# cheneeheng/2s-AGCN

Measured on AMD Instinct MI355X. Metric: skeleton-clips/sec fwd+bwd, NTU (N,3,300,25,2), higher is better.
Workload: dtype f32; 1 GPU; AGCN joint-stream NTU-xview shape, full training step (fwd, CE, bwd, grad all-reduce, clip 1.0, SGD nesterov); per_gpu_batch=64, global_batch=64, input=(N,3,300,25,2), parallelism=dp1, bn=per-replica

## Files before the change

2s-agcn_amd/csrc/adj_fused.hip:

```cpp
#include "agcn_common.h"
#include "split_f16.h"
#include "split_bf16.h"

namespace {

constexpr int CK = 16, NW = 8, NT = 512, WLR = 264, TP = 257;
constexpr int B_BYTES = 3 * 2 * WLR * 16;

struct AfArgs {
  const float* x;
  const unsigned short* wp;
  const float* bias;
  float* spart;
  float* tp_out;
  const float* dS;
  float* dtp;
  float* dbpart;
  int N, C, Ci, T, V, tt, ntiles, nchunks, nsb;
  int npl;
  int dbg;
  unsigned* x_absmax;
};

struct AfPackArgs {
  const float* w;
  unsigned short* wp;
  int M, K, nchunks;
};

template <int BM>
__global__ void __launch_bounds__(256) af_pack_kernel(const AfPackArgs p) {
  constexpr int PER_PLANE = 2 * BM * 8;
  const int ch = blockIdx.x % p.nchunks, sb = blockIdx.x / p.nchunks;
  unsigned short* dst = p.wp + (long)blockIdx.x * 3 * PER_PLANE;
  for (int e = threadIdx.x; e < PER_PLANE / 2; e += 256) {
    const int j = (e & 3) * 2;
    const int ml = (e >> 2) % BM;
    const int h = (e >> 2) / BM;
    const int m = sb * BM + ml;
    float v[2];
#pragma unroll
    for (int q = 0; q < 2; ++q) {
      const int kc = ch * CK + h * 8 + j + q;
      v[q] = (m < p.M && kc < p.K) ? p.w[(long)m * p.K + kc] : 0.f;
    }
    unsigned ph, pm, pl;
    sb_split_pair(v[0], v[1], ph, pm, pl);
    const int o = (h * BM + ml) * 8 + j;
    *reinterpret_cast<unsigned*>(dst + 0 * PER_PLANE + o) = ph;
    *reinterpret_cast<unsigned*>(dst + 1 * PER_PLANE + o) = pm;
    *reinterpret_cast<unsigned*>(dst + 2 * PER_PLANE + o) = pl;
  }
}

template <int TM, int NSUB, int MODE, int PD>
// ... 284 lines not shown
  const size_t stage = 2 * (a_bytes + B_BYTES);
  const int VP = 2 * ((V + 1) / 2);
  const size_t aux_f = (size_t)NW * V * V, aux_b = (size_t)2 * VP * 32 + 32;
  const size_t ph2 = ((size_t)32 * TP + (aux_f > aux_b ? aux_f : aux_b)) * 4;
  g.smem_bytes = ((stage > ph2 ? stage : ph2) + 15) & ~(size_t)15;
  g.pack_bytes = (size_t)g.nsb * g.nchunks * a_bytes;
  return g;
}

inline bool af_shape(int Ci, int& tm, int& nsub) {
  if (Ci == 16) { tm = 3; nsub = 3; return true; }
  if (Ci == 32) { tm = 2; nsub = 1; return true; }
  if (Ci == 64) { tm = 4; nsub = 1; return true; }
  return false;
}

template <int TM, int NSUB, int MODE, int PD>
int af_launch(AfArgs a, const AfGeom& g, hipStream_t s) {
  return agcn_launch_big<adj_fused_kernel<TM, NSUB, MODE, PD>>(dim3((unsigned)(a.N * g.ntiles * g.nsb)), dim3(NT),
                                                               g.smem_bytes, s, a);
}

template <int TM, int NSUB>
int af_pack(const float* wab, void* ws, int M, int K, const AfGeom& g, hipStream_t s) {
  AfPackArgs pk;
  pk.w = wab; pk.wp = (unsigned short*)ws; pk.M = M; pk.K = K; pk.nchunks = g.nchunks;
  hipLaunchKernelGGL((af_pack_kernel<TM * 32>), dim3(g.nsb * g.nchunks), dim3(256), 0, s, pk);
  return agcn_check_launch();
}

template <int TM, int NSUB>
int af_go(int mode, const AfArgs& a, const float* wab, void* ws, const AfGeom& g, hipStream_t s) {
  int rc = af_pack<TM, NSUB>(wab, ws, 6 * a.Ci, a.C, g, s);
  if (rc) return rc;
  const int pd = (g.nchunks % 4 == 0 && (TM <= 2 || g.nchunks >= 8)) ? 4 : (g.nchunks % 2 == 0 ? 2 : 1);
  if (pd == 4) return mode == 0 ? af_launch<TM, NSUB, 0, 4>(a, g, s) : af_launch<TM, NSUB, 1, 4>(a, g, s);
  if (pd == 2) return mode == 0 ? af_launch<TM, NSUB, 0, 2>(a, g, s) : af_launch<TM, NSUB, 1, 2>(a, g, s);
  return mode == 0 ? af_launch<TM, NSUB, 0, 1>(a, g, s) : af_launch<TM, NSUB, 1, 1>(a, g, s);
}

int af_run(int mode, AfArgs a, const float* wab, void* ws, size_t ws_bytes, hipStream_t s) {
  int tm, nsub;
  if (!af_shape(a.Ci, tm, nsub)) return AGCN_ERR_UNSUPPORTED;
  const AfGeom g = af_geometry(a.C, a.T, a.V, tm * 32, nsub);
  if (g.smem_bytes > 160 * 1024) return AGCN_ERR_UNSUPPORTED;
  if (g.pack_bytes > ws_bytes) return AGCN_ERR_WORKSPACE;
  a.tt = g.tt; a.ntiles = g.ntiles; a.nchunks = g.nchunks; a.nsb = g.nsb;
  a.wp = (const unsigned short*)ws;
  a.dbg = agcn_probe(AGCN_AF_DBG, nullptr);
  a.npl = agcn_npl();
  if (tm == 3) return af_go<3, 3>(mode, a, wab, ws, g, s);
  if (tm == 2) return af_go<2, 1>(mode, a, wab, ws, g, s);
  return af_go<4, 1>(mode, a, wab, ws, g, s);
}

bool af_supported(int C, int Ci, int T, int V) {
// ... 17 lines not shown
}

int agcn_adjacency_fused_fwd(const float* x, const float* wab, const float* bab, const float* A, const float* PA,
                             const float* alpha, float* tp_out, float* spart, float* P, float* adj, void* workspace,
                             size_t workspace_bytes, int N, int C, int Ci, int T, int V, void* stream) {
  return agcn_adjacency_fused_fwd_ex(x, wab, bab, A, PA, alpha, tp_out, spart, P, adj, nullptr, nullptr, workspace,
                                     workspace_bytes, N, C, Ci, T, V, stream);
}
int agcn_adjacency_fused_fwd_ex(const float* x, const float* wab, const float* bab, const float* A, const float* PA,
                                const float* alpha, float* tp_out, float* spart, float* P, float* adj, float* x_absmax_out,
                                const float* x_absmax_in, void* workspace, size_t workspace_bytes, int N, int C, int Ci, int T,
                                int V, void* stream) {
  if (!x || !wab || !PA || !spart || !P || !adj || !workspace || N <= 0 || C <= 0 || Ci <= 0 || T <= 0 || V <= 0 ||
      V > 32)
    return AGCN_ERR_ARG;
  if (!af_supported(C, Ci, T, V)) return AGCN_ERR_UNSUPPORTED;
  if (agcn_adj_ws_supported(N, C, Ci, T, V)) {
    const size_t img = agcn_adj_ws_workspace(C, Ci);
    if (workspace_bytes < img + 16) return AGCN_ERR_WORKSPACE;
    hipStream_t s = (hipStream_t)stream;
    const float* amax;
    void* slot = x_absmax_out ? (void*)x_absmax_out : static_cast<char*>(workspace) + img;
    if (int rc = agcn_operand_max(x_absmax_in, x, (long)N * C * T * V, slot, s, &amax)) return rc;
    if (x_absmax_in && x_absmax_out && x_absmax_out != x_absmax_in)
      if (hipMemcpyAsync(x_absmax_out, x_absmax_in, 4, hipMemcpyDeviceToDevice, s) != hipSuccess) return AGCN_ERR_ARG;
    const int tt = 256 / V > T ? T : 256 / V, slots = (T + tt - 1) / tt;
    int nused = 0;
    if (int rc = agcn_adj_ws_scores(x, wab, bab, tp_out, spart, slots, &nused, amax, workspace, img, N, C, Ci, T, V, s))
      return rc;
    return agcn_adj_finalize(spart, A, PA, alpha, P, adj, N, Ci, T, V, s, nused);
  }
  if (x_absmax_out && hipMemsetAsync(x_absmax_out, 0, 4, (hipStream_t)stream) != hipSuccess) return AGCN_ERR_ARG;
  AfArgs a = {};
  a.x_absmax = reinterpret_cast<unsigned*>(x_absmax_out);
  a.x = x; a.bias = bab; a.spart = spart; a.tp_out = tp_out;
  a.N = N; a.C = C; a.Ci = Ci; a.T = T; a.V = V;
  int rc = af_run(0, a, wab, workspace, workspace_bytes, (hipStream_t)stream);
  if (rc) return rc;
  return agcn_adj_finalize(spart, A, PA, alpha, P, adj, N, Ci, T, V, (hipStream_t)stream);
}

int agcn_adjacency_fused_bwd_scores(const float* x, const float* wab, const float* bab, const float* dS, float* dtp,
                                    float* dbpart, void* scratch, float* db, void* workspace, size_t workspace_bytes,
                                    int N, int C, int Ci, int T, int V, void* stream) {
  if (!x || !wab || !dS || !dtp || !dbpart || !scratch || !db || !workspace || N <= 0 || C <= 0 || Ci <= 0 ||
      T <= 0 || V <= 0 || V > 32)
    return AGCN_ERR_ARG;
  if (!af_supported(C, Ci, T, V)) return AGCN_ERR_UNSUPPORTED;
  AfArgs a = {};
  a.x = x; a.bias = bab; a.dS = dS; a.dtp = dtp; a.dbpart = dbpart;
  a.N = N; a.C = C; a.Ci = Ci; a.T = T; a.V = V;
  int rc = af_run(1, a, wab, workspace, workspace_bytes, (hipStream_t)stream);
  if (rc) return rc;
  const int tt = 256 / V > T ? T : 256 / V;
  return agcn_colsum(dbpart, N * ((T + tt - 1) / tt), 6 * Ci, scratch, db, stream);
// ... 4 lines not shown
```

2s-agcn_amd/csrc/adj_ws.hip:

```cpp
#include "agcn_common.h"
#include "split_f16.h"

namespace {

typedef __bf16 bf16x8 __attribute__((ext_vector_type(8)));
typedef unsigned u32x4 __attribute__((ext_vector_type(4)));

constexpr int AW_NW = 8, AW_NT = AW_NW * 64;

struct AwArgs {
  const float* x;
  const unsigned short* wp;
  const float* bias;
  float* spart;
  float* tp_out;
  const float* x_absmax;
  int N, C, Ci, T, V;
  int FT, nsplit, fper, slots;
};

struct AwPackArgs {
  const float* w;
  unsigned short* wp;
  int M, K, nks;
};

__global__ void __launch_bounds__(256) aw_pack_kernel(const AwPackArgs p) {
  const int e = blockIdx.x * 256 + threadIdx.x;
  if (e >= p.nks * 2 * p.M) return;
  const int m = e % p.M, h = (e / p.M) & 1, ks = e / (2 * p.M);
  u32x4 ph, pl;
#pragma unroll
  for (int e2 = 0; e2 < 4; ++e2) {
    float v[2];
#pragma unroll
    for (int q = 0; q < 2; ++q) {
      const int k = 16 * ks + 8 * h + 2 * e2 + q;
      v[q] = k < p.K ? p.w[(long)m * p.K + k] : 0.f;
    }
    unsigned a, b;
    split_pair_f16(v[0] * F16_W_SCALE, v[1] * F16_W_SCALE, a, b);
    ph[e2] = a; pl[e2] = b;
  }
  u32x4* dst = reinterpret_cast<u32x4*>(p.wp);
  dst[((long)(ks * 2 + 0) * 2 + h) * p.M + m] = ph;
  dst[((long)(ks * 2 + 1) * 2 + h) * p.M + m] = pl;
}

template <int TMS, int KS, int NSR, int TP>
__global__ void __launch_bounds__(AW_NT, 2) adj_ws_kernel(const AwArgs a) {
  constexpr int TM = 3 * TMS;
// ... 208 lines not shown
  AGCN_NOTE_KERNEL("adj_ws_kernel<%d, %d, %d, %d>", TMS, KS, NSR, TP);
  return rc;
}
template <int TMS, int KS, int NSR>
int aw_launch(const AwArgs& a, const AwGeom& g, hipStream_t s) {
  return g.TP == 252 ? aw_launch_tp<TMS, KS, NSR, 252>(a, g, s) : aw_launch_tp<TMS, KS, NSR, 256>(a, g, s);
}

}

static inline bool aw_enabled() {
  return agcn_knob(AGCN_ADJ_WS) != 0 && agcn_chain_f16x3();
}

bool agcn_adj_ws_supported(int N, int C, int Ci, int T, int V) {
  AwGeom g;
  return aw_enabled() && aw_geometry(N, C, Ci, T, V, g);
}

size_t agcn_adj_ws_workspace(int C, int Ci) { return (size_t)((C + 15) / 16) * 2 * 2 * (6 * Ci) * 16; }

int agcn_adj_ws_scores(const float* x, const float* wab, const float* bab, float* tp_out, float* spart, int slots,
                       int* nslots_used, const float* x_absmax, void* ws, size_t ws_bytes, int N, int C, int Ci, int T, int V,
                       hipStream_t s) {
  AwGeom g;
  if (!aw_geometry(N, C, Ci, T, V, g)) return AGCN_ERR_UNSUPPORTED;
  if (g.nsplit > slots) return AGCN_ERR_UNSUPPORTED;
  if (g.pack_bytes > ws_bytes) return AGCN_ERR_WORKSPACE;
  AwPackArgs pk;
  pk.w = wab; pk.wp = (unsigned short*)ws; pk.M = 6 * Ci; pk.K = C; pk.nks = g.ks;
  const int items = g.ks * 2 * 6 * Ci;
  hipLaunchKernelGGL(aw_pack_kernel, dim3((items + 255) / 256), dim3(256), 0, s, pk);
  int rc = agcn_check_launch();
  if (rc) return rc;
  AwArgs a = {};
  a.x = x; a.wp = (const unsigned short*)ws; a.bias = bab; a.spart = spart; a.tp_out = tp_out; a.x_absmax = x_absmax;
  a.N = N; a.C = C; a.Ci = Ci; a.T = T; a.V = V;
  a.FT = g.FT; a.nsplit = g.nsplit; a.fper = g.fper; a.slots = slots;
  *nslots_used = g.nsplit;
  if (g.tms == 1 && g.ks == 4) return g.nsr == 3 ? aw_launch<1, 4, 3>(a, g, s) : aw_launch<1, 4, 1>(a, g, s);
  if (g.tms == 2 && g.ks == 4) return aw_launch<2, 4, 1>(a, g, s);
  if (g.tms == 2 && g.ks == 8) return aw_launch<2, 8, 1>(a, g, s);
  return AGCN_ERR_UNSUPPORTED;
}
```

2s-agcn_amd/csrc/agcn_common.h:

```cpp
#pragma once
#include <hip/hip_runtime.h>
#include <stdint.h>
#include <stdlib.h>
#include <string.h>
#include "knobs.h"
#include "../../include/agcn_hip.h"

typedef float f32x16 __attribute__((ext_vector_type(16)));
typedef float f32x4 __attribute__((ext_vector_type(4)));

__device__ __forceinline__ f32x16 mfma32(float a, float b, f32x16 c) {
  return __builtin_amdgcn_mfma_f32_32x32x2f32(a, b, c, 0, 0, 0);
}
__device__ __forceinline__ int mfma_row(int j, int h) { return (j & 3) + 8 * (j >> 2) + 4 * h; }

__device__ __forceinline__ float mask_load(const float* m, long idx, int bits) {
  return bits ? m[idx >> 5] : m[idx];
}
__device__ __forceinline__ bool mask_pass(float raw, long idx, int bits) {
  return bits ? ((__builtin_bit_cast(unsigned, raw) >> (idx & 31)) & 1u) != 0u : raw > 0.f;
}

__device__ __forceinline__ float half_sum(float v) {
  v += __shfl_xor(v, 16);
  v += __shfl_xor(v, 8);
  v += __shfl_xor(v, 4);
  v += __shfl_xor(v, 2);
  v += __shfl_xor(v, 1);
  return v;
}

__device__ __forceinline__ int xcd_remap(int bid, int nwg) {
  const int q = nwg >> 3, r = nwg & 7, x = bid & 7, k = bid >> 3;
  const int base = (x < r) ? x * (q + 1) : r * (q + 1) + (x - r) * q;
  return base + k;
}

int agcn_adj_finalize(const float* spart, const float* A, const float* PA, const float* alpha, float* P, float* adj,
                      int N, int Ci, int T, int V, hipStream_t s, int nused = -1);

bool agcn_adj_ws_supported(int N, int C, int Ci, int T, int V);
size_t agcn_adj_ws_workspace(int C, int Ci);
int agcn_adj_ws_scores(const float* x, const float* wab, const float* bab, float* tp_out, float* spart, int slots,
                       int* nslots_used, const float* x_absmax, void* ws, size_t ws_bytes, int N, int C, int Ci, int T, int V,
                       hipStream_t s);

struct AgcnDryRun {
  long slab_slots;
  size_t ws_bytes;
};
static inline int agcn_dry_note(AgcnDryRun* d, long slab_slots, size_t ws_bytes) {
  if (slab_slots > d->slab_slots) d->slab_slots = slab_slots;
  if (ws_bytes > d->ws_bytes) d->ws_bytes = ws_bytes;
  return AGCN_OK;
}

static inline float* agcn_dry_present() { static float placeholder; return &placeholder; }

static inline bool agcn_sizes_ok(int N, int a, int b, int T, int V) {
  return N > 0 && a > 0 && b > 0 && T > 0 && V > 0 && V <= 32;
}

#include "tconv_plan.h"

bool agcn_bf16_conv_wide(int taps, int M);
enum AgcnTconvOp { AGCN_TCONV_FWD, AGCN_TCONV_BWD_DATA };
bool agcn_bf16_tconv_supported(AgcnTconvOp op, int taps, int stride, int pad);
struct GateArgs;
// ... 77 lines not shown
```

2s-agcn_amd/csrc/bn.hip:

```cpp
#include "agcn_common.h"

namespace {

constexpr int RG = 64;

__global__ void __launch_bounds__(256)
colsum_stage1_kernel(const float* __restrict__ X, int nslots, int W, int per_group, double* __restrict__ partial) {
  __shared__ double red[4][64];
  const int col = blockIdx.x * 64 + (threadIdx.x & 63), sub = threadIdx.x >> 6;
  const int g = blockIdx.y;
  const int s_end = min(nslots, (g + 1) * per_group);
  double acc = 0.0;
  if (col < W)
    for (int s = g * per_group + sub; s < s_end; s += 4) acc += (double)X[(long)s * W + col];
  red[sub][threadIdx.x & 63] = acc;
  __syncthreads();
  if (sub == 0 && col < W)
    partial[(long)g * W + col] = red[0][threadIdx.x] + red[1][threadIdx.x] + red[2][threadIdx.x] + red[3][threadIdx.x];
}

__global__ void colsum_stage2_kernel(const double* __restrict__ partial, int W, float* __restrict__ out) {
  const int col = blockIdx.x * blockDim.x + threadIdx.x;
  if (col >= W) return;
  double s = 0.0;
// ... 150 lines not shown
      dz = ((mb[e >> 5] >> (e & 31)) & 1u) ? dz : 0.f;
    }
    s0 += dz;
    s1 += dz * a[q];
    if (HAS2) s2 += dz * b[q];
  }
  s0 = half_sum(s0); s1 = half_sum(s1); s2 = half_sum(s2);
  s0 += __shfl_xor(s0, 32); s1 += __shfl_xor(s1, 32); s2 += __shfl_xor(s2, 32);
  const int wave = threadIdx.x >> 6;
  if ((threadIdx.x & 63) == 0) { red[0][wave] = s0; red[1][wave] = s1; red[2][wave] = s2; }
  __syncthreads();
  if (threadIdx.x < 3) {
    const int k = threadIdx.x;
    part[row * 3 + k] = red[k][0] + red[k][1] + red[k][2] + red[k][3];
  }
}

__global__ void bn_bwd_finalize_kernel(const float* __restrict__ part, int N, int C, double count, float pscale,
                                       const float* __restrict__ gamma1, const float* __restrict__ mean1,
                                       const float* __restrict__ invstd1, const float* __restrict__ gamma2,
                                       const float* __restrict__ mean2, const float* __restrict__ invstd2,
                                       float* __restrict__ coef, float* __restrict__ dgamma1,
                                       float* __restrict__ dbeta1, float* __restrict__ dgamma2,
                                       float* __restrict__ dbeta2) {
  const int c = blockIdx.x * blockDim.x + threadIdx.x;
  if (c >= C) return;
  double s0 = 0.0, s1 = 0.0, s2 = 0.0;
#pragma unroll 8
  for (int n = 0; n < N; ++n) {
    const float* p = part + ((long)n * C + c) * 3;
    s0 += (double)p[0]; s1 += (double)p[1]; s2 += (double)p[2];
  }
  {
    const double is = invstd1[c], mu = mean1[c], g = gamma1[c];
    const double sxh = is * (s1 - mu * s0);
    const double k = g * is;
    coef[0 * C + c] = (float)k;
    coef[1 * C + c] = (float)(-k * is * sxh / count);
    coef[2 * C + c] = (float)(-k * s0 / count + k * is * mu * sxh / count);
    dgamma1[c] = (float)sxh * pscale;
    dbeta1[c] = (float)s0 * pscale;
  }
  if (gamma2) {
    const double is = invstd2[c], mu = mean2[c], g = gamma2[c];
    const double sxh = is * (s2 - mu * s0);
    const double k = g * is;
    coef[3 * C + c] = (float)k;
    coef[4 * C + c] = (float)(-k * is * sxh / count);
// ... 146 lines not shown
  hipStream_t s = (hipStream_t)stream;
  if (y2) hipLaunchKernelGGL(bn_bwd_reduce_kernel<true>, dim3(N * C), dim3(256), 0, s, dout, (const float*)mask,
                             mask_bits, y1, y2, part, P);
  else hipLaunchKernelGGL(bn_bwd_reduce_kernel<false>, dim3(N * C), dim3(256), 0, s, dout, (const float*)mask,
                          mask_bits, y1, y2, part, P);
  return agcn_check_launch();
}

int agcn_bn_bwd_apply(const float* part, int nrows, double count, float param_grad_scale, const float* dout,
                      const void* mask, int mask_bits, const float* y1, const float* gamma1, const float* mean1, const float* invstd1,
                      const float* y2, const float* gamma2, const float* mean2, const float* invstd2, float* coef,
                      float* dy1, float* dgamma1, float* dbeta1, float* dy2, float* dgamma2, float* dbeta2, int N, int C,
                      int P, void* stream) {
  return agcn_bn_bwd_apply_ex(part, nrows, count, param_grad_scale, dout, mask, mask_bits, y1, gamma1, mean1, invstd1, y2,
                              gamma2, mean2, invstd2, coef, dy1, dgamma1, dbeta1, dy2, dgamma2, dbeta2, nullptr, N, C, P,
                              stream);
}

int agcn_bn_bwd_apply_ex(const float* part, int nrows, double count, float param_grad_scale, const float* dout,
                         const void* mask, int mask_bits, const float* y1, const float* gamma1, const float* mean1,
                         const float* invstd1, const float* y2, const float* gamma2, const float* mean2,
                         const float* invstd2, float* coef, float* dy1, float* dgamma1, float* dbeta1, float* dy2,
                         float* dgamma2, float* dbeta2, float* absmax1_out, int N, int C, int P, void* stream) {
  if (absmax1_out && hipMemsetAsync(absmax1_out, 0, 4, (hipStream_t)stream) != hipSuccess) return AGCN_ERR_ARG;
  if (!part || !dout || !y1 || !gamma1 || !mean1 || !invstd1 || !coef || !dy1 || !dgamma1 || !dbeta1 || nrows <= 0)
    return AGCN_ERR_ARG;
  if (y2 && (!gamma2 || !mean2 || !invstd2 || !dy2 || !dgamma2 || !dbeta2)) return AGCN_ERR_ARG;
  const long total = (long)N * C * P;
  if (total % 4 != 0 || total > 0xffffffffL) return AGCN_ERR_UNSUPPORTED;
  hipStream_t s = (hipStream_t)stream;
  hipLaunchKernelGGL(bn_bwd_finalize_kernel, dim3((C + 63) / 64), dim3(64), 0, s, part, nrows, C, count,
                     param_grad_scale, gamma1, mean1, invstd1, y2 ? gamma2 : nullptr, mean2, invstd2, coef, dgamma1,
                     dbeta1, dgamma2, dbeta2);
  int rc = agcn_check_launch();
  if (rc) return rc;
  const unsigned t4 = (unsigned)(total / 4);
  const dim3 g(ew_grid(t4)), b(256);
  if (y2)
    hipLaunchKernelGGL(bn_bwd_apply_kernel<true>, g, b, 0, s, (const float4*)dout, (const float4*)mask, mask_bits,
                       (const float4*)y1, (const float4*)y2, (const float*)coef, (float4*)dy1, (float4*)dy2, t4,
                       (unsigned)P, (unsigned)C, (unsigned*)absmax1_out);
  else
    hipLaunchKernelGGL(bn_bwd_apply_kernel<false>, g, b, 0, s, (const float4*)dout, (const float4*)mask, mask_bits,
                       (const float4*)y1, (const float4*)y2, (const float*)coef, (float4*)dy1, (float4*)dy2, t4,
                       (unsigned)P, (unsigned)C, (unsigned*)absmax1_out);
  return agcn_check_launch();
}

int agcn_bn_bwd(const float* dout, const void* mask, int mask_bits, const float* y1, const float* gamma1,
                const float* mean1, const float* invstd1, const float* y2, const float* gamma2, const float* mean2,
                const float* invstd2, float* part, float* coef, float* dy1, float* dgamma1, float* dbeta1, float* dy2,
                float* dgamma2, float* dbeta2, int N, int C, int P, void* stream) {
  int rc = agcn_bn_bwd_reduce(dout, mask, mask_bits, y1, y2, part, N, C, P, stream);
  if (rc) return rc;
  return agcn_bn_bwd_apply(part, N, (double)N * (double)P, 1.0f, dout, mask, mask_bits, y1, gamma1, mean1, invstd1, y2, gamma2,
                           mean2, invstd2, coef, dy1, dgamma1, dbeta1, dy2, dgamma2, dbeta2, N, C, P, stream);
// ... 7 lines not shown
```

2s-agcn_amd/csrc/wgrad9_bf16.hip:

```cpp
#include "agcn_common.h"
#include "split_bf16.h"
#include "split_f16.h"

namespace {

constexpr int TC = 80;
constexpr int DP = 84;
constexpr int XW = TC + 8;
constexpr int XPB = 88;

struct TrArgs {
  const float* in;
  float* out;
  int N, R, T, V, Tp, S;
  const float* absmax;
  long plane;
};

template <bool F16, int RB, int TT, int FPL>
__global__ void __launch_bounds__(256) tv_transpose_kernel(const TrArgs a) {
  extern __shared__ __attribute__((aligned(16))) float tile[];
  static_assert(FPL == 4 || (F16 && FPL == 8), "a lane writes one 16-byte store per plane");
  constexpr int QL = TT / FPL, NSUB = 64 / QL;
  const int S = a.S;
  const int ntt = (a.Tp * S + TT - 1) / TT, nrb = (a.R + RB - 1) / RB;
// ... 49 lines not shown
        const int f = (FPL * q + j) * S + par;
        val[j] = (f < tl) ? tile[r * pitch + f * a.V + v] : 0.f;
      }
      const long o = ((((long)n * a.V + v) * a.R + r0 + r) * S + par) * a.Tp + t0 / S + FPL * q;
      if constexpr (F16) {
        unsigned hh[FPL / 2], ll[FPL / 2];
#pragma unroll
        for (int j = 0; j < FPL / 2; ++j) split_pair_f16_mix(val[2 * j] * rs_s, val[2 * j + 1] * rs_s, hh[j], ll[j]);
        unsigned short* oh = reinterpret_cast<unsigned short*>(a.out);
        if constexpr (FPL == 8) {
          *reinterpret_cast<u32x4*>(oh + o) = u32x4{hh[0], hh[1], hh[2], hh[3]};
          *reinterpret_cast<u32x4*>(oh + a.plane + o) = u32x4{ll[0], ll[1], ll[2], ll[3]};
        } else {
          *reinterpret_cast<uint2*>(oh + o) = make_uint2(hh[0], hh[1]);
          *reinterpret_cast<uint2*>(oh + a.plane + o) = make_uint2(ll[0], ll[1]);
        }
      } else {
        *reinterpret_cast<f32x4*>(a.out + o) = f32x4{val[0], val[1], val[2], val[3]};
      }
    }
  }
}

struct W9Args {
  const float* dyT;
  const float* xT;
  float* part;
  int N, M, C, V, T, Tp;
  int nchunk, units, units_per_split, ncb;
  int npl;
  const unsigned short* dyH;
  const unsigned short* xH;
  long dy_plane, x_plane;
  const float* dy_absmax;
  const float* x_absmax;
};

template <int S>
__device__ __forceinline__ bf16x8 window_frag(const unsigned (&p)[8]) {
  u32x4 r;
  if (S % 2 == 0) {
#pragma unroll
    for (int i = 0; i < 4; ++i) r[i] = p[S / 2 + i];
  } else {
#pragma unroll
    for (int i = 0; i < 4; ++i) r[i] = __builtin_amdgcn_alignbit(p[(S + 1) / 2 + i], p[(S - 1) / 2 + i], 16);
// ... 329 lines not shown
inline W9Geom w9_geometry(int N, int M, int C, int V, int T, int stride, int taps = 9, int Tx = 0) {
  W9Geom g;
  g.rt = (M % 128 == 0) ? 4 : 2;
  const int BM = g.rt * 32, CBW = (4 / g.rt) * 32;
  g.Tp = ((Tx > T ? Tx : T) + 7) & ~7;
  g.nchunk = (T + TC - 1) / TC;
  g.units = N * V * g.nchunk;
  g.nmb = (M + BM - 1) / BM;
  g.ncb = (C + CBW - 1) / CBW;
  const int tiles = g.nmb * g.ncb;
  int want = 512 / tiles;
  if (want < 1) want = 1;
  if (want > g.units) want = g.units;
  g.units_per_split = (g.units + want - 1) / want;
  g.nsplit = (g.units + g.units_per_split - 1) / g.units_per_split;
  g.slab_bytes = (size_t)g.nsplit * taps * M * C * 4;
  g.dyT_bytes = (size_t)N * V * M * g.Tp * 4;
  g.xT_bytes = (size_t)N * V * C * stride * g.Tp * 4;
  g.smem_bytes = (size_t)BM * DP * 4 + (size_t)3 * stride * CBW * XPB * 2;
  g.smem_f16 = (size_t)2 * BM * DPH * 2 + (size_t)2 * stride * CBW * XPB * 2;
  return g;
}

int w9_transpose(const float* in, float* out, int N, int R, int T, int V, int Tp, int S, hipStream_t s,
                 const float* absmax = nullptr) {
  TrArgs t;
  t.in = in; t.out = out; t.N = N; t.R = R; t.T = T; t.V = V; t.Tp = Tp; t.S = S;
  t.absmax = absmax; t.plane = (long)N * V * R * S * Tp;
  if (absmax) {
    const int rem = T % 128;
    if (T <= 128 || rem == 0 || rem > 64) {
      constexpr int RB = 4, TT = 128;
      const int ntt = (Tp * S + TT - 1) / TT, nrb = (R + RB - 1) / RB;
      const size_t smem = (size_t)RB * (TT * V + 4) * 4;
      hipLaunchKernelGGL((tv_transpose_kernel<true, RB, TT, 8>), dim3((unsigned)(N * nrb * ntt)), dim3(256), smem, s, t);
    } else {
      constexpr int RB = 8, TT = 64;
      const int ntt = (Tp * S + TT - 1) / TT, nrb = (R + RB - 1) / RB;
      const size_t smem = (size_t)RB * (TT * V + 4) * 4;
      hipLaunchKernelGGL((tv_transpose_kernel<true, RB, TT, 8>), dim3((unsigned)(N * nrb * ntt)), dim3(256), smem, s, t);
    }
  } else {
    const int ntt = (Tp * S + 63) / 64, nrb = (R + 7) / 8;
    const size_t smem = (size_t)8 * (64 * V + 4) * 4;
    hipLaunchKernelGGL((tv_transpose_kernel<false, 8, 64, 4>), dim3((unsigned)(N * nrb * ntt)), dim3(256), smem, s, t);
  }
  return agcn_check_launch();
}

template <int RT, int CT, int STRIDE, int TAPS = 9, int SH0 = 0>
int w9_launch_f16(const W9Args& a, const W9Geom& g, hipStream_t s) {
  if (TAPS == 9) AGCN_NOTE_KERNEL("wgrad9_f16_kernel<%d, %d, %d>", RT, CT, STRIDE);
  else AGCN_NOTE_KERNEL("wgrad9_f16_kernel<%d, %d, %d, %d, %d>", RT, CT, STRIDE, TAPS, SH0);
  return agcn_launch_big<wgrad9_f16_kernel<RT, CT, STRIDE, TAPS, SH0>>(dim3((unsigned)(g.nmb * g.ncb), (unsigned)g.nsplit),
                                                                       dim3(256), g.smem_f16, s, a);
}

template <int RT, int CT, int STRIDE>
int w9_launch(const W9Args& a, const W9Geom& g, hipStream_t s) {
  AGCN_NOTE_KERNEL("wgrad9_bf16_kernel<%d, %d, %d>", RT, CT, STRIDE);
  return agcn_launch_big<wgrad9_bf16_kernel<RT, CT, STRIDE>>(dim3((unsigned)(g.nmb * g.ncb), (unsigned)g.nsplit), dim3(256),
                                                             g.smem_bytes, s, a);
}

template <int TAPS, int SH0>
int w9_launch_taps(const W9Args& a, const W9Geom& g, hipStream_t s) {
  return g.rt == 4 ? w9_launch_f16<4, 1, 1, TAPS, SH0>(a, g, s) : w9_launch_f16<2, 2, 1, TAPS, SH0>(a, g, s);
}

inline bool w9_f16x3() { return agcn_knob(AGCN_WGRAD9_F16X3) != 0; }

int w9_run(const float* dy, const float* x, void* ws, size_t ws_bytes, int* nslabs, int N, int M, int C, int V, int T,
           int taps, int stride, int pad, bool f16, const float* dy_absmax, const float* x_absmax, hipStream_t s,
           AgcnDryRun* dry) {
  const int To = (T + 2 * pad - taps) / stride + 1;
  if (To < 1 || (taps != 9 && !f16)) return AGCN_ERR_UNSUPPORTED;
  const W9Geom g = w9_geometry(N, M, C, V, To, stride, taps, taps == 9 ? 0 : T);
  const size_t bytes = g.slab_bytes + g.dyT_bytes + g.xT_bytes + 512;
  if (dry) return agcn_dry_note(dry, 0, bytes);
  if (bytes > ws_bytes) return AGCN_ERR_WORKSPACE;
  unsigned char* base = (unsigned char*)ws;
  float* dyT = (float*)(base + ((g.slab_bytes + 255) & ~(size_t)255));
  float* xT = (float*)((unsigned char*)dyT + g.dyT_bytes);
  if ((size_t)((unsigned char*)xT - base) + g.xT_bytes + 8 > ws_bytes) return AGCN_ERR_WORKSPACE;
  if (f16) {
    unsigned* scr = reinterpret_cast<unsigned*>((unsigned char*)xT + g.xT_bytes);
    if (int rc = agcn_operand_max(dy_absmax, dy, (long)N * M * To * V, scr, s, &dy_absmax)) return rc;
    if (int rc = agcn_operand_max(x_absmax, x, (long)N * C * T * V, scr + 1, s, &x_absmax)) return rc;
  }
  int rc = w9_transpose(dy, dyT, N, M, To, V, g.Tp, 1, s, f16 ? dy_absmax : nullptr);
  if (rc) return rc;
  rc = w9_transpose(x, xT, N, C, T, V, g.Tp, stride, s, f16 ? x_absmax : nullptr);
  if (rc) return rc;
  W9Args a = {};
  a.dyT = dyT; a.xT = xT; a.part = (float*)ws;
  a.N = N; a.M = M; a.C = C; a.V = V; a.T = To; a.Tp = g.Tp;
  a.nchunk = g.nchunk; a.units = g.units; a.units_per_split = g.units_per_split; a.ncb = g.ncb;
  a.npl = agcn_npl();
  *nslabs = g.nsplit;
  if (!f16) {
    if (stride == 2) return w9_launch<4, 1, 2>(a, g, s);
    return g.rt == 4 ? w9_launch<4, 1, 1>(a, g, s) : w9_launch<2, 2, 1>(a, g, s);
  }
  a.dyH = reinterpret_cast<const unsigned short*>(dyT);
  a.xH = reinterpret_cast<const unsigned short*>(xT);
  a.dy_plane = (long)N * V * M * g.Tp;
  a.x_plane = (long)N * V * C * stride * g.Tp;
  a.dy_absmax = dy_absmax; a.x_absmax = x_absmax;
  if (taps == 9) {
    if (stride == 2) return w9_launch_f16<4, 1, 2>(a, g, s);
    return g.rt == 4 ? w9_launch_f16<4, 1, 1>(a, g, s) : w9_launch_f16<2, 2, 1>(a, g, s);
  }
  switch (taps * 16 + 4 - pad) {
    case 3 * 16 + 3: return w9_launch_taps<3, 3>(a, g, s);
    case 3 * 16 + 4: return w9_launch_taps<3, 4>(a, g, s);
    case 5 * 16 + 2: return w9_launch_taps<5, 2>(a, g, s);
// ... 10 lines not shown
bool agcn_wgrad9_bf16_supported(int M, int C, int V, int stride) {
  if (M % 64 != 0 || C % 64 != 0 || V < 1 || V > 32 || !agcn_chained()) return false;
  return stride == 1 || (stride == 2 && M % 128 == 0);
}

int agcn_wgrad9_bf16(const float* dy, const float* x, void* ws, size_t ws_bytes, int* nslabs, int N, int M, int C, int V,
                     int T, int stride, hipStream_t s, const float* dy_absmax, const float* x_absmax, AgcnDryRun* dry) {
  return w9_run(dy, x, ws, ws_bytes, nslabs, N, M, C, V, T, 9, stride, 4, agcn_npl() == 3 && w9_f16x3(), dy_absmax,
                x_absmax, s, dry);
}

bool agcn_wgrad_tconv_f16_supported(int M, int C, int V, int taps, int stride, int pad) {
  if (stride != 1 || (taps != 3 && taps != 5 && taps != 7) || pad < 0 || pad > (taps - 1) / 2 || taps - pad > 5)
    return false;
  return agcn_gemm_precision() == 3 && w9_f16x3() && M % 64 == 0 && C % 64 == 0 && V >= 1 && V <= 32;
}

int agcn_wgrad_tconv_f16(const float* dy, const float* x, void* ws, size_t ws_bytes, int* nslabs, int N, int M, int C,
                         int V, int T, int taps, int pad, hipStream_t s, const float* dy_absmax, const float* x_absmax,
                         AgcnDryRun* dry) {
  if (!agcn_wgrad_tconv_f16_supported(M, C, V, taps, 1, pad)) return AGCN_ERR_UNSUPPORTED;
  return w9_run(dy, x, ws, ws_bytes, nslabs, N, M, C, V, T, taps, 1, pad, true, dy_absmax, x_absmax, s, dry);
}
```

include/agcn_hip.h:

```cpp
#ifndef AGCN_HIP_H
#define AGCN_HIP_H

#include <stddef.h>

#ifdef __cplusplus
extern "C" {
#endif

#define AGCN_OK 0
#define AGCN_ERR_ARG (-1)
#define AGCN_ERR_WORKSPACE (-2)
#define AGCN_ERR_UNSUPPORTED (-3)

int agcn_version(void);
const char* agcn_arch(void);

const char* agcn_last_kernel(void);
const char* agcn_gemm_mode(void);
const char* agcn_chain_mode(void);

int agcn_conv_tile_frames(int V, int T_out);
int agcn_conv_num_tiles(int V, int T_out);
int agcn_conv_stats_tiles(int Cin, int Cout, int T_out, int V, int taps, int stride);
int agcn_scores_num_tiles(int V, int T);
// ... 45 lines not shown
                                   const float* x_absmax, void* stream);
int agcn_absmax(const float* x, long n, float* out, void* stream);
int agcn_conv_fwd_ex(const float* x, const float* w, const float* bias, float* y, float* stats_part, void* workspace,
                     size_t workspace_bytes, int N, int Cin, int Cout, int T, int V, int taps, int stride,
                     const float* x_absmax, void* stream);
int agcn_conv_bwd_data_ex(const float* dy, const float* w, float* dx, int accumulate, const float* add1,
                          const float* mask1, const float* add2, const float* mask2, void* workspace,
                          size_t workspace_bytes, int N, int Cin, int Cout, int T, int V, int taps, int stride,
                          const float* dy_absmax, void* stream);

size_t agcn_tconv_workspace(int Cin, int Cout, int T, int V, int taps, int stride, int pad);
int agcn_tconv_stats_tiles(int Cin, int Cout, int T_out, int V, int taps, int stride, int pad);
int agcn_tconv_fwd(const float* x, const float* w, const float* bias, float* y, float* stats_part, void* workspace,
                   size_t workspace_bytes, int N, int Cin, int Cout, int T, int V, int taps, int stride, int pad,
                   const float* x_absmax, void* stream);
int agcn_tconv_bwd_data(const float* dy, const float* w, float* dx, int accumulate, const float* add1,
                        const float* mask1, const float* add2, const float* mask2, void* workspace,
                        size_t workspace_bytes, int N, int Cin, int Cout, int T, int V, int taps, int stride, int pad,
                        const float* dy_absmax, void* stream);
size_t agcn_tconv_bwd_weight_workspace(int N, int Cin, int Cout, int T, int V, int taps, int stride, int pad);
int agcn_tconv_bwd_weight(const float* dy, const float* x, float* dw, void* workspace, size_t workspace_bytes, int N,
                          int Cin, int Cout, int T, int V, int taps, int stride, int pad, const float* dy_absmax,
                          const float* x_absmax, void* stream);

int agcn_gcn_first_supported(int C, int Cout, int V);
int agcn_gcn_first_tiles(int T, int V);
int agcn_gcn_first_fwd(const float* x, const float* adj, const float* wcat, const float* bias, const float* wdown,
                       const float* bdown, float* ypre, float* ystats, float* dpre, float* dstats, int N, int C, int Cout,
                       int T, int V, void* stream);

size_t agcn_gcn_unit_infer_workspace(int C, int Cout, int K2, int T, int V);
int agcn_gcn_unit_infer(const float* x, const float* adj, const float* wcat, const float* bias, const float* res,
                        const float* x2, const float* w2, int K2, int relu, float* y, void* workspace,
                        size_t workspace_bytes, int N, int C, int Cout, int T, int V, void* stream);
int agcn_conv9_infer(const float* x, const float* w, const float* bias, const float* res, int relu, float* y,
                     void* workspace, size_t workspace_bytes, int N, int Cin, int Cout, int T, int V, int stride,
                     void* stream);

int agcn_tconv_infer(const float* x, const float* w, const float* bias, const float* a_s, const float* a_t,
                     const float* a_c, const float* res, int relu, float* y, void* workspace, size_t workspace_bytes,
                     int N, int Cin, int Cout, int T, int V, int taps, int stride, int pad, const float* x_absmax,
                     void* stream);

int agcn_gcn_aggregate_project_bwd_data(const float* dy, const float* adj, const float* wcat, float* dx,
                                        int accumulate, const float* add1, const float* mask1, const float* add2,
                                        const float* mask2, int mask_bits, void* workspace, size_t workspace_bytes, int N, int C,
// ... 181 lines not shown
```

Baseline: 1025 clips/s.

## Fold small memset/memcpy into kernels and add row-staged paired wgrad transpose

The 4-byte absmax memset and memcpy calls are moved into existing pack and BN-finalize kernels, which removes several tiny stream operations per step. Separately, a new row-staged transpose kernel loads whole operand rows into LDS with global_load_lds DMA, then writes the f16-split transposed layout. When both dy and x qualify, the two operands are handled in one launch. A public entry point and a planner header are added as well, bringing more code paths and alignment conditions that have to hold.

```diff
diff --git a/2s-agcn_amd/csrc/adj_fused.hip b/2s-agcn_amd/csrc/adj_fused.hip
--- a/2s-agcn_amd/csrc/adj_fused.hip
+++ b/2s-agcn_amd/csrc/adj_fused.hip
@@ -26,11 +26,13 @@
   const float* w;
   unsigned short* wp;
   int M, K, nchunks;
+  unsigned* zero_word;
 };
 
 template <int BM>
 __global__ void __launch_bounds__(256) af_pack_kernel(const AfPackArgs p) {
   constexpr int PER_PLANE = 2 * BM * 8;
+  if (p.zero_word && blockIdx.x == 0 && threadIdx.x == 0) *p.zero_word = 0u;
   const int ch = blockIdx.x % p.nchunks, sb = blockIdx.x / p.nchunks;
   unsigned short* dst = p.wp + (long)blockIdx.x * 3 * PER_PLANE;
   for (int e = threadIdx.x; e < PER_PLANE / 2; e += 256) {
@@ -361,16 +363,16 @@
 }
 
 template <int TM, int NSUB>
-int af_pack(const float* wab, void* ws, int M, int K, const AfGeom& g, hipStream_t s) {
+int af_pack(const float* wab, void* ws, int M, int K, const AfGeom& g, unsigned* zero_word, hipStream_t s) {
   AfPackArgs pk;
-  pk.w = wab; pk.wp = (unsigned short*)ws; pk.M = M; pk.K = K; pk.nchunks = g.nchunks;
+  pk.w = wab; pk.wp = (unsigned short*)ws; pk.M = M; pk.K = K; pk.nchunks = g.nchunks; pk.zero_word = zero_word;
   hipLaunchKernelGGL((af_pack_kernel<TM * 32>), dim3(g.nsb * g.nchunks), dim3(256), 0, s, pk);
   return agcn_check_launch();
 }
 
 template <int TM, int NSUB>
 int af_go(int mode, const AfArgs& a, const float* wab, void* ws, const AfGeom& g, hipStream_t s) {
-  int rc = af_pack<TM, NSUB>(wab, ws, 6 * a.Ci, a.C, g, s);
+  int rc = af_pack<TM, NSUB>(wab, ws, 6 * a.Ci, a.C, g, a.x_absmax, s);
   if (rc) return rc;
   const int pd = (g.nchunks % 4 == 0 && (TM <= 2 || g.nchunks >= 8)) ? 4 : (g.nchunks % 2 == 0 ? 2 : 1);
   if (pd == 4) return mode == 0 ? af_launch<TM, NSUB, 0, 4>(a, g, s) : af_launch<TM, NSUB, 1, 4>(a, g, s);
@@ -434,15 +436,14 @@
     const float* amax;
     void* slot = x_absmax_out ? (void*)x_absmax_out : static_cast<char*>(workspace) + img;
     if (int rc = agcn_operand_max(x_absmax_in, x, (long)N * C * T * V, slot, s, &amax)) return rc;
-    if (x_absmax_in && x_absmax_out && x_absmax_out != x_absmax_in)
-      if (hipMemcpyAsync(x_absmax_out, x_absmax_in, 4, hipMemcpyDeviceToDevice, s) != hipSuccess) return AGCN_ERR_ARG;
+    float* hand_on = (x_absmax_in && x_absmax_out && x_absmax_out != x_absmax_in) ? x_absmax_out : nullptr;
     const int tt = 256 / V > T ? T : 256 / V, slots = (T + tt - 1) / tt;
     int nused = 0;
-    if (int rc = agcn_adj_ws_scores(x, wab, bab, tp_out, spart, slots, &nused, amax, workspace, img, N, C, Ci, T, V, s))
+    if (int rc = agcn_adj_ws_scores(x, wab, bab, tp_out, spart, slots, &nused, amax, workspace, img, N, C, Ci, T, V, s,
+                                    hand_on))
       return rc;
     return agcn_adj_finalize(spart, A, PA, alpha, P, adj, N, Ci, T, V, s, nused);
   }
-  if (x_absmax_out && hipMemsetAsync(x_absmax_out, 0, 4, (hipStream_t)stream) != hipSuccess) return AGCN_ERR_ARG;
   AfArgs a = {};
   a.x_absmax = reinterpret_cast<unsigned*>(x_absmax_out);
   a.x = x; a.bias = bab; a.spart = spart; a.tp_out = tp_out;
diff --git a/2s-agcn_amd/csrc/adj_ws.hip b/2s-agcn_amd/csrc/adj_ws.hip
--- a/2s-agcn_amd/csrc/adj_ws.hip
+++ b/2s-agcn_amd/csrc/adj_ws.hip
@@ -23,10 +23,13 @@
   const float* w;
   unsigned short* wp;
   int M, K, nks;
+  const float* copy_from;
+  float* copy_to;
 };
 
 __global__ void __launch_bounds__(256) aw_pack_kernel(const AwPackArgs p) {
   const int e = blockIdx.x * 256 + threadIdx.x;
+  if (p.copy_to && e == 0) *p.copy_to = *p.copy_from;
   if (e >= p.nks * 2 * p.M) return;
   const int m = e % p.M, h = (e / p.M) & 1, ks = e / (2 * p.M);
   u32x4 ph, pl;
@@ -281,13 +284,14 @@
 
 int agcn_adj_ws_scores(const float* x, const float* wab, const float* bab, float* tp_out, float* spart, int slots,
                        int* nslots_used, const float* x_absmax, void* ws, size_t ws_bytes, int N, int C, int Ci, int T, int V,
-                       hipStream_t s) {
+                       hipStream_t s, float* x_absmax_copy) {
   AwGeom g;
   if (!aw_geometry(N, C, Ci, T, V, g)) return AGCN_ERR_UNSUPPORTED;
   if (g.nsplit > slots) return AGCN_ERR_UNSUPPORTED;
   if (g.pack_bytes > ws_bytes) return AGCN_ERR_WORKSPACE;
   AwPackArgs pk;
   pk.w = wab; pk.wp = (unsigned short*)ws; pk.M = 6 * Ci; pk.K = C; pk.nks = g.ks;
+  pk.copy_from = x_absmax; pk.copy_to = x_absmax_copy;
   const int items = g.ks * 2 * 6 * Ci;
   hipLaunchKernelGGL(aw_pack_kernel, dim3((items + 255) / 256), dim3(256), 0, s, pk);
   int rc = agcn_check_launch();
diff --git a/2s-agcn_amd/csrc/agcn_common.h b/2s-agcn_amd/csrc/agcn_common.h
--- a/2s-agcn_amd/csrc/agcn_common.h
+++ b/2s-agcn_amd/csrc/agcn_common.h
@@ -43,7 +43,7 @@
 size_t agcn_adj_ws_workspace(int C, int Ci);
 int agcn_adj_ws_scores(const float* x, const float* wab, const float* bab, float* tp_out, float* spart, int slots,
                        int* nslots_used, const float* x_absmax, void* ws, size_t ws_bytes, int N, int C, int Ci, int T, int V,
-                       hipStream_t s);
+                       hipStream_t s, float* x_absmax_copy = nullptr);
 
 struct AgcnDryRun {
   long slab_slots;
diff --git a/2s-agcn_amd/csrc/bn.hip b/2s-agcn_amd/csrc/bn.hip
--- a/2s-agcn_amd/csrc/bn.hip
+++ b/2s-agcn_amd/csrc/bn.hip
@@ -196,8 +196,9 @@
                                        const float* __restrict__ mean2, const float* __restrict__ invstd2,
                                        float* __restrict__ coef, float* __restrict__ dgamma1,
                                        float* __restrict__ dbeta1, float* __restrict__ dgamma2,
-                                       float* __restrict__ dbeta2) {
+                                       float* __restrict__ dbeta2, unsigned* zero_word) {
   const int c = blockIdx.x * blockDim.x + threadIdx.x;
+  if (zero_word && c == 0) *zero_word = 0u;
   if (c >= C) return;
   double s0 = 0.0, s1 = 0.0, s2 = 0.0;
 #pragma unroll 8
@@ -390,7 +391,6 @@
                          const float* invstd1, const float* y2, const float* gamma2, const float* mean2,
                          const float* invstd2, float* coef, float* dy1, float* dgamma1, float* dbeta1, float* dy2,
                          float* dgamma2, float* dbeta2, float* absmax1_out, int N, int C, int P, void* stream) {
-  if (absmax1_out && hipMemsetAsync(absmax1_out, 0, 4, (hipStream_t)stream) != hipSuccess) return AGCN_ERR_ARG;
   if (!part || !dout || !y1 || !gamma1 || !mean1 || !invstd1 || !coef || !dy1 || !dgamma1 || !dbeta1 || nrows <= 0)
     return AGCN_ERR_ARG;
   if (y2 && (!gamma2 || !mean2 || !invstd2 || !dy2 || !dgamma2 || !dbeta2)) return AGCN_ERR_ARG;
@@ -399,7 +399,7 @@
   hipStream_t s = (hipStream_t)stream;
   hipLaunchKernelGGL(bn_bwd_finalize_kernel, dim3((C + 63) / 64), dim3(64), 0, s, part, nrows, C, count,
                      param_grad_scale, gamma1, mean1, invstd1, y2 ? gamma2 : nullptr, mean2, invstd2, coef, dgamma1,
-                     dbeta1, dgamma2, dbeta2);
+                     dbeta1, dgamma2, dbeta2, (unsigned*)absmax1_out);
   int rc = agcn_check_launch();
   if (rc) return rc;
   const unsigned t4 = (unsigned)(total / 4);
diff --git a/2s-agcn_amd/csrc/tv_plan.h b/2s-agcn_amd/csrc/tv_plan.h
--- /dev/null
+++ b/2s-agcn_amd/csrc/tv_plan.h
@@ -0,0 +1,82 @@
+#pragma once
+#include <stddef.h>
+
+#define TV_ROUTE_AUTO (-1)
+#define TV_ROUTE_TILED 0
+#define TV_ROUTE_ROWS 1
+#define TV_LDS_BUDGET (64 * 1024)
+
+struct TvPlan {
+  int route;
+  int RB;
+  int TT;
+  int FPL;
+  int nrb, ntt;
+  long grid;
+  size_t lds_bytes;
+  bool dma16;
+};
+
+struct TvBlock {
+  int n, r0, rows;
+  int t0, frames;
+  long src_off;
+  long run_floats;
+};
+
+inline bool tv_rows_applies(int T, int V, bool f16) {
+  return f16 && (size_t)T * V * 4 <= (size_t)TV_LDS_BUDGET;
+}
+
+inline TvBlock tv_plan_block(const TvPlan& p, int R, int T, int V, long b) {
+  TvBlock k = {};
+  const int tti = (int)(b % p.ntt);
+  b /= p.ntt;
+  const int rbi = (int)(b % p.nrb);
+  k.n = (int)(b / p.nrb);
+  k.r0 = rbi * p.RB;
+  k.rows = R - k.r0 < p.RB ? R - k.r0 : p.RB;
+  k.t0 = tti * p.TT;
+  k.frames = T - k.t0 < 0 ? 0 : (T - k.t0 < p.TT ? T - k.t0 : p.TT);
+  k.src_off = (((long)k.n * R + k.r0) * T + k.t0) * V;
+  k.run_floats = p.route == TV_ROUTE_ROWS ? (long)k.rows * T * V : 0;
+  return k;
+}
+
+inline TvPlan tv_plan(int N, int R, int T, int V, int Tp, int S, bool f16, unsigned base_misalign,
+                      int route = TV_ROUTE_AUTO) {
+  TvPlan p = {};
+  if (route == TV_ROUTE_AUTO) route = tv_rows_applies(T, V, f16) ? TV_ROUTE_ROWS : TV_ROUTE_TILED;
+  p.route = route;
+  p.FPL = f16 ? 8 : 4;
+  if (route == TV_ROUTE_ROWS) {
+    const size_t row = (size_t)T * V * 4;
+    p.RB = 8;
+    while (p.RB > 1 && p.RB * row > (size_t)TV_LDS_BUDGET) p.RB >>= 1;
+    if (p.RB > R) {
+      p.RB = 1;
+      while (p.RB < R) p.RB <<= 1;
+    }
+    p.TT = T;
+    p.nrb = (R + p.RB - 1) / p.RB;
+    p.ntt = 1;
+    p.lds_bytes = (p.RB * row + 15) & ~(size_t)15;
+    p.dma16 = base_misalign == 0;
+    for (int n = 0; n < (N < 2 ? N : 2) && p.dma16; ++n)
+      for (int rbi = 0; rbi < p.nrb && p.dma16; ++rbi) {
+        const TvBlock k = tv_plan_block(p, R, T, V, (long)n * p.nrb + rbi);
+        p.dma16 = (k.src_off & 3) == 0 && (k.run_floats & 3) == 0;
+      }
+  } else {
+    const int rem = T % 128;
+    const bool wide_tile = f16 && (T <= 128 || rem == 0 || rem > 64);
+    p.RB = wide_tile ? 4 : 8;
+    p.TT = wide_tile ? 128 : 64;
+    p.nrb = (R + p.RB - 1) / p.RB;
+    p.ntt = (Tp * S + p.TT - 1) / p.TT;
+    p.lds_bytes = (size_t)p.RB * (p.TT * V + 4) * 4;
+    p.dma16 = false;
+  }
+  p.grid = (long)N * p.nrb * p.ntt;
+  return p;
+}
diff --git a/2s-agcn_amd/csrc/wgrad9_bf16.hip b/2s-agcn_amd/csrc/wgrad9_bf16.hip
--- a/2s-agcn_amd/csrc/wgrad9_bf16.hip
+++ b/2s-agcn_amd/csrc/wgrad9_bf16.hip
@@ -1,6 +1,7 @@
 #include "agcn_common.h"
 #include "split_bf16.h"
 #include "split_f16.h"
+#include "tv_plan.h"
 
 namespace {
 
@@ -96,6 +97,72 @@
   }
 }
 
+struct TvRowsRec {
+  const float* in;
+  unsigned short* out;
+  const float* absmax;
+  long plane;
+  int R, T, V, Tp, S, RB, nrb, dma16;
+};
+struct TvRowsArgs {
+  TvRowsRec rec[2];
+  int nblk0;
+};
+
+__global__ void __launch_bounds__(256) tv_rows_kernel(const TvRowsArgs args) {
+  extern __shared__ __attribute__((aligned(16))) float tile[];
+  int b = xcd_remap((int)blockIdx.x, (int)gridDim.x);
+  const bool second = b >= args.nblk0;
+  if (second) b -= args.nblk0;
+  const TvRowsRec& a = args.rec[second ? 1 : 0];
+  const int S = a.S, V = a.V, T = a.T, Tp = a.Tp;
+  const int rbi = b % a.nrb, n = b / a.nrb;
+  const int r0 = rbi * a.RB, rows = min(a.RB, a.R - r0);
+  const int E = T * V;
+  const int L = rows * E;
+  const float* src = a.in + ((long)n * a.R + r0) * E;
+  const int lane = threadIdx.x & 63;
+  const int wave = __builtin_amdgcn_readfirstlane(threadIdx.x >> 6);
+  typedef const __attribute__((address_space(1))) void* gptr_t;
+  typedef __attribute__((address_space(3))) void* lptr_t;
+  if (a.dma16) {
+    for (int e0 = wave * 256; e0 < L; e0 += 1024)
+      if (e0 + 4 * lane < L) __builtin_amdgcn_global_load_lds((gptr_t)(src + e0 + 4 * lane), (lptr_t)(tile + e0), 16, 0, 0);
+  } else {
+    for (int e0 = wave * 64; e0 < L; e0 += 256)
+      if (e0 + lane < L) __builtin_amdgcn_global_load_lds((gptr_t)(src + e0 + lane), (lptr_t)(tile + e0), 4, 0, 0);
+  }
+  __syncthreads();
+  float rs_s = 1.f, rs_inv = 1.f;
+  f16_range_scale(a.absmax, rs_s, rs_inv);
+  (void)rs_inv;
+  const int Tq = Tp >> 3;
+  const int gpr = S * Tq;
+  const int G = rows * gpr;
+  const int ngb = (G + 7) >> 3, nvb = (V + 7) >> 3;
+  const int vj = (lane >> 2) & 7, gl = (lane & 3) + 4 * (lane >> 5);
+  for (int it = wave; it < nvb * ngb; it += 4) {
+    const int vb = it / ngb, gb = it - vb * ngb;
+    const int v = vb * 8 + vj, g = gb * 8 + gl;
+    if (v < V && g < G) {
+      const int r = g / gpr, rem = g - r * gpr;
+      const int par = rem / Tq, q = rem - par * Tq;
+      float val[8];
+#pragma unroll
+      for (int j = 0; j < 8; ++j) {
+        const int f = (8 * q + j) * S + par;
+        val[j] = (f < T) ? tile[r * E + f * V + v] : 0.f;
+      }
+      const long o = ((((long)n * V + v) * a.R + r0 + r) * S + par) * Tp + 8 * q;
+      unsigned hh[4], ll[4];
+#pragma unroll
+      for (int j = 0; j < 4; ++j) split_pair_f16_mix(val[2 * j] * rs_s, val[2 * j + 1] * rs_s, hh[j], ll[j]);
+      *reinterpret_cast<u32x4*>(a.out + o) = u32x4{hh[0], hh[1], hh[2], hh[3]};
+      *reinterpret_cast<u32x4*>(a.out + a.plane + o) = u32x4{ll[0], ll[1], ll[2], ll[3]};
+    }
+  }
+}
+
 struct W9Args {
   const float* dyT;
   const float* xT;
@@ -471,29 +538,58 @@
   return g;
 }
 
-int w9_transpose(const float* in, float* out, int N, int R, int T, int V, int Tp, int S, hipStream_t s,
-                 const float* absmax = nullptr) {
+struct TvOperand {
+  const float* in;
+  float* out;
+  int R, T, S;
+  const float* absmax;
+};
+
+inline TvPlan w9_tv_plan(const TvOperand& o, int N, int V, int Tp, int route = TV_ROUTE_AUTO) {
+  return tv_plan(N, o.R, o.T, V, Tp, o.S, o.absmax != nullptr, (unsigned)(reinterpret_cast<unsigned long>(o.in) & 15),
+                 route);
+}
+
+inline TvRowsRec w9_rows_rec(const TvOperand& o, const TvPlan& p, int N, int V, int Tp) {
+  TvRowsRec r;
+  r.in = o.in; r.out = reinterpret_cast<unsigned short*>(o.out); r.absmax = o.absmax;
+  r.plane = (long)N * V * o.R * o.S * Tp;
+  r.R = o.R; r.T = o.T; r.V = V; r.Tp = Tp; r.S = o.S; r.RB = p.RB; r.nrb = p.nrb; r.dma16 = p.dma16 ? 1 : 0;
+  return r;
+}
+
+int w9_transpose(const TvOperand& o, int N, int V, int Tp, hipStream_t s, int route = TV_ROUTE_AUTO) {
+  const TvPlan p = w9_tv_plan(o, N, V, Tp, route);
+  if (p.grid > 0x7fffffffL) return AGCN_ERR_UNSUPPORTED;
+  if (p.route == TV_ROUTE_ROWS) {
+    TvRowsArgs a;
+    a.rec[0] = a.rec[1] = w9_rows_rec(o, p, N, V, Tp);
+    a.nblk0 = (int)p.grid;
+    hipLaunchKernelGGL(tv_rows_kernel, dim3((unsigned)p.grid), dim3(256), p.lds_bytes, s, a);
+    return agcn_check_launch();
+  }
   TrArgs t;
-  t.in = in; t.out = out; t.N = N; t.R = R; t.T = T; t.V = V; t.Tp = Tp; t.S = S;
-  t.absmax = absmax; t.plane = (long)N * V * R * S * Tp;
-  if (absmax) {
-    const int rem = T % 128;
-    if (T <= 128 || rem == 0 || rem > 64) {
-      constexpr int RB = 4, TT = 128;
-      const int ntt = (Tp * S + TT - 1) / TT, nrb = (R + RB - 1) / RB;
-      const size_t smem = (size_t)RB * (TT * V + 4) * 4;
-      hipLaunchKernelGGL((tv_transpose_kernel<true, RB, TT, 8>), dim3((unsigned)(N * nrb * ntt)), dim3(256), smem, s, t);
-    } else {
-      constexpr int RB = 8, TT = 64;
-      const int ntt = (Tp * S + TT - 1) / TT, nrb = (R + RB - 1) / RB;
-      const size_t smem = (size_t)RB * (TT * V + 4) * 4;
-      hipLaunchKernelGGL((tv_transpose_kernel<true, RB, TT, 8>), dim3((unsigned)(N * nrb * ntt)), dim3(256), smem, s, t);
-    }
-  } else {
-    const int ntt = (Tp * S + 63) / 64, nrb = (R + 7) / 8;
-    const size_t smem = (size_t)8 * (64 * V + 4) * 4;
-    hipLaunchKernelGGL((tv_transpose_kernel<false, 8, 64, 4>), dim3((unsigned)(N * nrb * ntt)), dim3(256), smem, s, t);
-  }
+  t.in = o.in; t.out = o.out; t.N = N; t.R = o.R; t.T = o.T; t.V = V; t.Tp = Tp; t.S = o.S;
+  t.absmax = o.absmax; t.plane = (long)N * V * o.R * o.S * Tp;
+  const dim3 grid((unsigned)p.grid);
+  if (!o.absmax) hipLaunchKernelGGL((tv_transpose_kernel<false, 8, 64, 4>), grid, dim3(256), p.lds_bytes, s, t);
+  else if (p.TT == 128) hipLaunchKernelGGL((tv_transpose_kernel<true, 4, 128, 8>), grid, dim3(256), p.lds_bytes, s, t);
+  else hipLaunchKernelGGL((tv_transpose_kernel<true, 8, 64, 8>), grid, dim3(256), p.lds_bytes, s, t);
+  return agcn_check_launch();
+}
+
+int w9_transpose_pair(const TvOperand& dy, const TvOperand& x, int N, int V, int Tp, hipStream_t s) {
+  const TvPlan pd = w9_tv_plan(dy, N, V, Tp), px = w9_tv_plan(x, N, V, Tp);
+  if (pd.route != TV_ROUTE_ROWS || px.route != TV_ROUTE_ROWS || pd.grid + px.grid > 0x7fffffffL) {
+    if (int rc = w9_transpose(dy, N, V, Tp, s)) return rc;
+    return w9_transpose(x, N, V, Tp, s);
+  }
+  TvRowsArgs a;
+  a.rec[0] = w9_rows_rec(dy, pd, N, V, Tp);
+  a.rec[1] = w9_rows_rec(x, px, N, V, Tp);
+  a.nblk0 = (int)pd.grid;
+  hipLaunchKernelGGL(tv_rows_kernel, dim3((unsigned)(pd.grid + px.grid)), dim3(256),
+                     pd.lds_bytes > px.lds_bytes ? pd.lds_bytes : px.lds_bytes, s, a);
   return agcn_check_launch();
 }
 
@@ -537,10 +633,9 @@
     if (int rc = agcn_operand_max(dy_absmax, dy, (long)N * M * To * V, scr, s, &dy_absmax)) return rc;
     if (int rc = agcn_operand_max(x_absmax, x, (long)N * C * T * V, scr + 1, s, &x_absmax)) return rc;
   }
-  int rc = w9_transpose(dy, dyT, N, M, To, V, g.Tp, 1, s, f16 ? dy_absmax : nullptr);
-  if (rc) return rc;
-  rc = w9_transpose(x, xT, N, C, T, V, g.Tp, stride, s, f16 ? x_absmax : nullptr);
-  if (rc) return rc;
+  const TvOperand tdy = {dy, dyT, M, To, 1, f16 ? dy_absmax : nullptr};
+  const TvOperand tx = {x, xT, C, T, stride, f16 ? x_absmax : nullptr};
+  if (int rc = w9_transpose_pair(tdy, tx, N, V, g.Tp, s)) return rc;
   W9Args a = {};
   a.dyT = dyT; a.xT = xT; a.part = (float*)ws;
   a.N = N; a.M = M; a.C = C; a.V = V; a.T = To; a.Tp = g.Tp;
@@ -597,3 +692,13 @@
   if (!agcn_wgrad_tconv_f16_supported(M, C, V, taps, 1, pad)) return AGCN_ERR_UNSUPPORTED;
   return w9_run(dy, x, ws, ws_bytes, nslabs, N, M, C, V, T, taps, 1, pad, true, dy_absmax, x_absmax, s, dry);
 }
+
+int agcn_tv_transpose(const float* in, void* out, int N, int R, int T, int V, int Tp, int S, const float* absmax,
+                      int route, void* stream) {
+  if (!in || !out || !absmax || N < 1 || R < 1 || T < 1 || V < 1 || V > 32 || S < 1 || Tp < 8) return AGCN_ERR_ARG;
+  if ((Tp & 7) != 0 || (long)Tp * S < T || (reinterpret_cast<unsigned long>(out) & 15) != 0) return AGCN_ERR_ARG;
+  if (route < TV_ROUTE_AUTO || route > TV_ROUTE_ROWS) return AGCN_ERR_ARG;
+  if (route == TV_ROUTE_ROWS && !tv_rows_applies(T, V, true)) return AGCN_ERR_UNSUPPORTED;
+  const TvOperand o = {in, static_cast<float*>(out), R, T, S, absmax};
+  return w9_transpose(o, N, V, Tp, (hipStream_t)stream, route);
+}
diff --git a/include/agcn_hip.h b/include/agcn_hip.h
--- a/include/agcn_hip.h
+++ b/include/agcn_hip.h
@@ -91,6 +91,8 @@
 int agcn_tconv_bwd_weight(const float* dy, const float* x, float* dw, void* workspace, size_t workspace_bytes, int N,
                           int Cin, int Cout, int T, int V, int taps, int stride, int pad, const float* dy_absmax,
                           const float* x_absmax, void* stream);
+int agcn_tv_transpose(const float* in, void* out, int N, int R, int T, int V, int Tp, int S, const float* absmax,
+                      int route, void* stream);
 
 int agcn_gcn_first_supported(int C, int Cout, int V);
 int agcn_gcn_first_tiles(int T, int V);
```

Measured after the change: 1035 clips/s, median of 6. About the same (+0.9%).
